# AechPro/rlgym-ppo

Hardware: AMD Instinct MI355X
Metric: ppo_update_samples_per_sec (higher is better)
Workload: dtype f32; 1 GPU; configs[1]: 4096 agents x 128 steps = 524,288-sample buffer, obs 107 f32, 90 discrete actions, 256x3 policy + critic; batch 524,288, minibatch 65,536

## Files before the change

rlgym_ppo_amd/csrc/api.hip:

```cpp
#include "build_id.h"
#include <math.h>
#include <stdarg.h>
#include <string.h>

#include "common.hpp"

namespace rlppo {

static thread_local char g_err[512] = "";

void set_error(const char *fmt, ...) {
    va_list ap;
    va_start(ap, fmt);
    vsnprintf(g_err, sizeof(g_err), fmt, ap);
    va_end(ap);
}

static int64_t padded_width(int64_t d) {
    const int64_t p16 = round_up(d, 16), p64 = round_up(d, 64);
    return (p64 - p16) * 10 >= p64 ? p16 : p64;
}
static int64_t padded_out(int64_t d) {
    if (d <= 32) return 32;
    if (d <= 64) return 64;
// ... 546 lines not shown
}

int64_t rlppo_act_done_words(int64_t n) { return n > 0 ? cdiv(n, 16) : 0; }

size_t rlppo_gae_workspace_bytes(int64_t n) { return gae_workspace_bytes(n) + 256; }

int rlppo_gae(void *stream, const float *rews, const float *dones, const float *truncated, const float *values, int64_t n,
              double gamma, double lmbda, float return_std, float *value_targets, float *advantages, float *returns,
              void *workspace, size_t ws_bytes) {
    if (n == 0) return 0;
    RLPPO_CHECK_ARG(n > 0 && rews && dones && truncated && values && value_targets && advantages && returns && workspace,
                    "gae: bad argument");
    return launch_gae((hipStream_t)stream, rews, dones, truncated, values, n, gamma, lmbda, return_std, value_targets,
                      advantages, returns, workspace, ws_bytes);
}

static int g_two_streams = 1;
static int g_fused_gather = 1;
static int g_update_bf16 = 0;
struct SlotBank {
    hipStream_t main[RLPPO_MAX_SLOTS] = {}, side[RLPPO_MAX_SLOTS] = {};
    hipEvent_t ev_fork[RLPPO_MAX_SLOTS] = {}, ev_join[RLPPO_MAX_SLOTS] = {}, ev_slot[RLPPO_MAX_SLOTS] = {}, ev_mid[RLPPO_MAX_SLOTS] = {};
    bool pending[RLPPO_MAX_SLOTS] = {};
};
static SlotBank g_banks[64];
static int slot_bank(SlotBank **bank) {
    int dev = 0;
    RLPPO_HIP(hipGetDevice(&dev));
    RLPPO_CHECK_ARG(dev >= 0 && dev < 64, "device id %d", dev);
    *bank = &g_banks[dev];
    return 0;
}
static int ensure_slot(SlotBank &b, int s) {
    if (!b.side[s]) {
        RLPPO_HIP(hipStreamCreateWithFlags(&b.side[s], hipStreamNonBlocking));
        RLPPO_HIP(hipStreamCreateWithFlags(&b.main[s], hipStreamNonBlocking));
        RLPPO_HIP(hipEventCreateWithFlags(&b.ev_fork[s], hipEventDisableTiming));
        RLPPO_HIP(hipEventCreateWithFlags(&b.ev_join[s], hipEventDisableTiming));
        RLPPO_HIP(hipEventCreateWithFlags(&b.ev_slot[s], hipEventDisableTiming));
        RLPPO_HIP(hipEventCreateWithFlags(&b.ev_mid[s], hipEventDisableTiming));
    }
    return 0;
}
static int order_after(hipStream_t to, hipStream_t from, hipEvent_t ev) {
    RLPPO_HIP(hipEventRecord(ev, from));
    RLPPO_HIP(hipStreamWaitEvent(to, ev, 0));
    return 0;
}

static size_t tn_layer_floats(const NetLayout &net, int l, int64_t mb, int prec) {
    size_t f = tn_partial_floats(net.L[l].out, net.L[l].in, mb);
    if (net.L[l].out == 1) {
        const size_t g = (size_t)cdiv(mb, 64) * (size_t)(net.L[l].pin + 4);
        if (g > f) f = g;
    }
    if (prec == 1 && l == net.n_layers - 1) {
        const size_t g = thin_dw_ws_floats(net.L[l].out, net.L[l].pin, mb);
        if (g > f) f = g;
    }
    return (f + 3) / 4 * 4;
}
static size_t tn_ws_floats(const NetLayout &net, int64_t mb, int prec) {
    size_t m = 0;
// ... 606 lines not shown
        rc = order_after(p.st, caller, bk.ev_slot[slot]);
        if (rc) return rc;
        bk.pending[slot] = true;
    }
    rc = gather(p);
    if (rc) return rc;
    p.side = p.st;
    if (g_two_streams) {
        p.side = bk.side[slot];
        rc = order_after(p.side, p.st, bk.ev_fork[slot]);
        if (rc) return rc;
    }
    ++g_cnt_pass;
    if (twin) ++g_cnt_paired_pass;
    if (p.rows.rowtab) ++g_cnt_gather_fused_pass;
    rc = twin ? paired_pass(p, bk, slot) : two_chain_pass(p);
    if (rc) return rc;
    if (!twin && p.side != p.st) {
        rc = order_after(p.st, p.side, bk.ev_join[slot]);
        if (rc) return rc;
    }
    if (p.defer && dws.n) {
        ++g_cnt_group_dw;
        rc = launch_gemm_tn_group(p.st, dws.p, dws.n, mb, p.w.pol.tn, p.w.tn_floats);
    }
    return rc;
}

int rlppo_ppo_join(void *stream) {
    SlotBank *bank = nullptr;
    int rc = slot_bank(&bank);
    if (rc) return rc;
    SlotBank &bk = *bank;
    for (int s = 1; s < RLPPO_MAX_SLOTS; ++s)
        if (bk.pending[s]) {
            rc = order_after((hipStream_t)stream, bk.main[s], bk.ev_slot[s]);
            if (rc) return rc;
            bk.pending[s] = false;
        }
    return 0;
}

int rlppo_clip_adam(void *stream, float *params, float *grads, float *exp_avg, float *exp_avg_sq, int64_t n,
                    double max_norm, double lr, double beta1, double beta2, double eps, int64_t step, double *gnorm2) {
    if (n == 0) return 0;
    RLPPO_CHECK_ARG(n > 0 && params && grads && exp_avg && exp_avg_sq && gnorm2 && step >= 1, "clip_adam: bad argument");
    const double bc1 = 1.0 - pow(beta1, (double)step);
// ... 146 lines not shown
    ++g_selection_epoch;
    return 0;
}
int rlppo_dbg_set(int32_t key, int32_t value) {
    ++g_selection_epoch;
    switch (key) {
        case 1: set_gae_algo(value); return 0;
        case 4: g_two_streams = value; return 0;
        case 21: set_gae_spin_limit(value); return 0;
        case 22: set_gae_oversubscribe(value); return 0;
        case 34: set_fused_spin_limit(value); return 0;
        case 35: set_fused_test_hold(value); return 0;
        case 36: set_split_persistent(value); return 0;
        case 23: set_b16_wide_tiles(value); return 0;
        case 24: set_exp_fast_transform(value); return 0;
        case 26: g_fused_gather = value; return 0;
        case 27: g_fused_act = value; return 0;
        case 29: g_paired = value; return 0;
        case 31: g_head_order = value; return 0;
        case 32: g_fold_vhead = value; return 0;
        case 33: set_pair_interleave(value); return 0;
        case 37: g_group_dw = value; return 0;
        case 38: set_tn_group_budget(value); return 0;
        case 40: set_nt_skinny(value); return 0;
        case 41: g_window_mode = value; return 0;
        default: break;
    }
    set_error("dbg_set: unknown key %d", key);
    return RLPPO_ERR_ARG;
}
int64_t rlppo_selection_epoch(void) { return g_selection_epoch; }
const int64_t *rlppo_selection_epoch_ptr(void) { return &g_selection_epoch; }
int64_t rlppo_dbg_counter(int32_t key) {
    switch (key) {
        case 0: return g_cnt_fused_act;
        case 1: return g_cnt_act_chain;
        case 2: return g_cnt_pass;
        case 3: return g_cnt_paired_pass;
        case 4: return g_cnt_gather_fused_pass;
        case 5: return g_cnt_group_dw;
        default: return -1;
    }
}
size_t rlppo_dbg_gemm_nt_bits_bytes(int64_t M, int32_t N) { return nt_bits_floats(M, N) * sizeof(float); }
int rlppo_dbg_gemm_nt_bits(void *stream, const float *A, int64_t lda, const float *B, int64_t ldb, const float *bias, float *C,
                           int64_t ldc, int64_t M, int32_t N, int32_t K, int32_t epilogue, void *bits) {
// ... 34 lines not shown
                            (float *)ws, ws_bytes / sizeof(float));
    return rc == -1 ? RLPPO_ERR_ARG : rc;
}
static int tn_products(const rlppo_tn_product *p, int32_t n, TnProduct *q) {
    RLPPO_CHECK_ARG(p && n > 0 && n <= 2 * RLPPO_MAX_LAYERS, "gemm_tn_group: %d products (1..%d)", n, 2 * RLPPO_MAX_LAYERS);
    for (int i = 0; i < n; ++i) {
        q[i].dY = p[i].dY; q[i].ldy = p[i].ldy; q[i].ny_valid = p[i].ny_valid; q[i].X = p[i].X; q[i].ldx = p[i].ldx;
        q[i].kx_valid = p[i].kx_valid; q[i].dW = p[i].dW; q[i].db = p[i].db; q[i].out = p[i].out; q[i].in = p[i].in;
        q[i].rowtab = p[i].rowtab; q[i].src_rows = p[i].src_rows;
    }
    return 0;
}
size_t rlppo_dbg_gemm_tn_group_workspace_bytes(const rlppo_tn_product *p, int32_t n, int64_t M) {
    if (!p || n <= 0 || n > 2 * RLPPO_MAX_LAYERS) return 0;
    int outs[2 * RLPPO_MAX_LAYERS], ins[2 * RLPPO_MAX_LAYERS];
    for (int i = 0; i < n; ++i) {
        outs[i] = p[i].out;
        ins[i] = p[i].in;
    }
    return tn_group_floats(outs, ins, n, M) * sizeof(float);
}
int rlppo_dbg_gemm_tn_group(void *stream, const rlppo_tn_product *p, int32_t n, int64_t M, void *ws, size_t ws_bytes) {
    TnProduct q[2 * RLPPO_MAX_LAYERS];
    const int rc = tn_products(p, n, q);
    if (rc) return rc;
    return launch_gemm_tn_group((hipStream_t)stream, q, n, M, (float *)ws, ws_bytes / sizeof(float));
}
size_t rlppo_dbg_gemm_tn_workspace_bytes(int32_t out, int32_t in, int64_t M) { return tn_partial_floats(out, in, M) * sizeof(float); }
int rlppo_dbg_gemm_tn(void *stream, const float *dY, int64_t ldy, int32_t ny_valid, const float *X, int64_t ldx,
                      int32_t kx_valid, float *dW, float *db, int32_t out, int32_t in, int64_t M, void *ws, size_t ws_bytes) {
    return launch_gemm_tn((hipStream_t)stream, dY, ldy, ny_valid, X, ldx, kx_valid, dW, db, out, in, M, (float *)ws,
                          ws_bytes / sizeof(float));
}
}
```

rlgym_ppo_amd/csrc/common.hpp:

```cpp
#pragma once
#include <hip/hip_runtime.h>
#include <stdint.h>
#include <stdio.h>

#include <atomic>

#include "../../include/rlppo.h"

namespace rlppo {

void set_error(const char *fmt, ...);

#define RLPPO_CHECK_ARG(cond, ...)                \
    do {                                          \
        if (!(cond)) {                            \
            rlppo::set_error(__VA_ARGS__);        \
            return RLPPO_ERR_ARG;                 \
        }                                         \
    } while (0)

#define RLPPO_HIP(expr)                                                                         \
    do {                                                                                        \
        hipError_t e_ = (expr);                                                                 \
        if (e_ != hipSuccess) {                                                                 \
// ... 84 lines not shown
void set_infer_bf16(int v);
void set_pair_interleave(int v);
void set_nt_skinny(int on);
int get_infer_bf16();
size_t tn_partial_floats(int out, int in, int64_t M);
int launch_gemm_tn(hipStream_t st, const float *dY, int64_t ldy, int ny_valid, const float *X, int64_t ldx, int kx_valid,
                   float *dW, float *db, int out, int in, int64_t M, float *ws, size_t ws_floats, const unsigned *rowtab = nullptr,
                   int64_t src_rows = 0, const TnPair *pair = nullptr);
bool tn_gather_ok(int64_t ldx, int64_t src_rows);
struct TnProduct {
    const float *dY = nullptr;
    int64_t ldy = 0;
    int ny_valid = 0;
    const float *X = nullptr;
    int64_t ldx = 0;
    int kx_valid = 0;
    float *dW = nullptr, *db = nullptr;
    int out = 0, in = 0;
    const unsigned *rowtab = nullptr;
    int64_t src_rows = 0;
};
constexpr int TN_GROUP_MAX = 2 * RLPPO_MAX_LAYERS;
size_t tn_group_floats(const int *outs, const int *ins, int n, int64_t M);
int launch_gemm_tn_group(hipStream_t st, const TnProduct *prods, int n, int64_t M, float *ws, size_t ws_floats);
void set_tn_group_budget(int workgroups);

bool nt_b16_ok(int N, int K, bool hidden);
bool nt_split_ok(int N, int K);
void set_split_persistent(int v);
int launch_pack_split(hipStream_t st, const float *S, int64_t ld, int R, int Cc, unsigned short *planes);
int launch_gemm_nt_split(hipStream_t st, const float *A, int64_t lda, const unsigned short *planes, const float *bias, float *C, int64_t ldc,
                         int64_t M, int N, int K, int mode, unsigned long long *bits);
int launch_gemm_nt_b16(hipStream_t st, const unsigned short *A, int64_t lda, const unsigned short *B, int64_t ldb, const float *bias,
                       float *C, int64_t ldc, unsigned short *Cb, int64_t ldcb, int64_t M, int N, int K, int epi, int mode,
                       unsigned long long *bits);
void set_b16_wide_tiles(int on);
bool tn_b16_ok(int pout, int pin);
int launch_gemm_tn_b16(hipStream_t st, const unsigned short *dY, int64_t ldy, const unsigned short *X, int64_t ldx, float *dW,
                       float *db, int pout, int pin, int out, int in, int64_t M, float *ws, size_t ws_floats);

void set_exp_fast_transform(int on);

bool gemv_head_ok(int out, int kp);
int launch_gemv_fwd(hipStream_t st, const float *x, int64_t ldx, const float *w, const float *b, float *y, int64_t ldy, int64_t n, int kp, int pout);
int launch_gemv_fwd_b16(hipStream_t st, const unsigned short *x, int64_t ldx, const float *w, const float *b, float *y, int64_t ldy,
                        int64_t n, int kp, int pout);
bool thin_head_ok(int out, int kp);
// ... 119 lines not shown
```

rlgym_ppo_amd/csrc/gemm.hip:

```cpp
#include "gemm_detail.hpp"

namespace rlppo {

template <int NB, int EPI, int BKT, bool BITS = false, bool GATHER = false>
__global__ __launch_bounds__(256, BKT == 16 ? 4 : 2) void gemm_nt_dma_kernel(const float *__restrict__ A, unsigned lda_b,
                                                                              const float *__restrict__ B, unsigned ldb_b,
                                                                              const float *__restrict__ bias,
                                                                              const float *__restrict__ mask_src,
                                                                              unsigned ldm_b, float *__restrict__ C,
                                                                              unsigned ldc_b, int64_t M, int K,
                                                                              unsigned long long *__restrict__ bits = nullptr,
                                                                              const unsigned *__restrict__ rowtab = nullptr,
                                                                              unsigned src_rows = 0, NtAlt alt = NtAlt{},
                                                                              NtDot dot = NtDot{}, NtDot dot_alt = NtDot{}) {
    constexpr int BN = NB * 16;
    constexpr int CPR = BKT / 4;
    constexpr int RPW = 64 / CPR;
    constexpr int RPP = 4 * RPW;
    constexpr int A_IT = SBM / RPP, B_IT = BN / RPP;
    constexpr int B_REM = BN % RPP;
    static_assert(B_REM % RPW == 0, "the ragged staging pass must be whole wave instructions");
    __shared__ __attribute__((aligned(16))) float lds[2 * SBM * BKT + 2 * BN * BKT];
    float *As = lds;
    float *Bs = lds + 2 * SBM * BKT;
// ... 461 lines not shown
        case 4: return launch_nt_1<4>(st, grid, epi, A, la, B, lb, bias, mask_src, lm, C, lc, M, K);
        default: return launch_nt_1<2>(st, grid, epi, A, la, B, lb, bias, mask_src, lm, C, lc, M, K);
    }
}

namespace {
constexpr int TM = 32;
constexpr unsigned OOR = 0x80000000u;
}

struct TnGeom {
    int ni, nj, wn;
    __host__ __device__ int bnt() const { return wn * ni * 16; }
    __host__ __device__ int bkx() const { return (4 / wn) * nj * 16; }
    __host__ __device__ int tile_floats() const { return ni * nj * 1024; }
};
static TnGeom tn_geometry(int out, int in) {
    if (in > 96 && in <= 112) return TnGeom{2, 7, 4};
    if (out > 64 && out <= 96) return TnGeom{3, 4, 2};
    return TnGeom{4, 4, 2};
}

constexpr int TN_LDS_FLOATS = 2 * 2 * 32 * 128;
template <int TMT, int NI, int NJ, int WN, bool GATHER>
__device__ __forceinline__ void tn_tile(float *lds, const float *__restrict__ dY, unsigned ldy_b, int ny_valid,
                                        const float *__restrict__ X, unsigned ldx_b, int kx_valid, bool with_db, int out, int64_t M,
                                        int rows_per_wg, float *__restrict__ partial, const unsigned *__restrict__ rowtab,
                                        unsigned src_rows, int bx, int by, int bz, int tiles_x, int tiles_y, int splits_z) {
    constexpr int WK = 4 / WN;
    constexpr int BNT = WN * NI * 16, BKX = WK * NJ * 16, TILE_F = NI * NJ * 1024;
    constexpr int PPW = TMT / 8;
    static_assert(2 * 2 * TMT * 128 <= TN_LDS_FLOATS && 8 * 128 <= TN_LDS_FLOATS, "stage buffers");
    float *Ys = lds;
    float *Xs = lds + 2 * TMT * 128;

    const int tid = threadIdx.x;
    const int lane = tid & 63, wave = tid >> 6;
    const int wave_u = __builtin_amdgcn_readfirstlane(wave);
    const int r16 = lane & 15, q = lane >> 4;
    const int wn = wave / WK, wk = wave % WK;
    const int n0 = bx * BNT, k0 = by * BKX;
    const int64_t mbeg = (int64_t)bz * rows_per_wg;
    const int rows = (int)((M - mbeg) < rows_per_wg ? (M - mbeg) : rows_per_wg);
    const int steps = (rows + TMT - 1) / TMT;
    const int rem = rows - (steps - 1) * TMT;
    const int ny_here = (ny_valid - n0) < BNT ? (ny_valid - n0) : BNT;
    const int kx_here = (kx_valid - k0) < BKX ? (kx_valid - k0) : BKX;

    const __amdgpu_buffer_rsrc_t y_rs = make_rsrc(reinterpret_cast<const char *>(dY) + mbeg * ldy_b + (int64_t)n0 * 4,
                                                  (unsigned)(rows - 1) * ldy_b + (unsigned)ny_here * 4);
    const __amdgpu_buffer_rsrc_t x_rs =
// ... 82 lines not shown
        for (int c = 0; c < TMT / 16; ++c) {
#pragma unroll
            for (int s = 0; s < 4; ++s) {
                const int m = c * 16 + s * 4;
                float fa[NI], fb[NJ];
#pragma unroll
                for (int i = 0; i < NI; ++i) fa[i] = Yc[m * 128 + fy[i]];
#pragma unroll
                for (int j = 0; j < NJ; ++j) fb[j] = Xc[m * 128 + fx[j]];
#pragma unroll
                for (int i = 0; i < NI; ++i)
#pragma unroll
                    for (int j = 0; j < NJ; ++j) {
                        if (c & 1) acc2[i][j] = MFMA16(fa[i], fb[j], acc2[i][j]);
                        else acc[i][j] = MFMA16(fa[i], fb[j], acc[i][j]);
                    }
            }
        }
        __builtin_amdgcn_sched_barrier(0);
        asm volatile("s_waitcnt vmcnt(0)" ::: "memory");
        if (more && (st + 2) == steps && rem < TMT) clear_tail(cur ^ 1);
        __syncthreads();
    }

    if (want_db) {
        float *red = lds;
        const int lcol = ((tid & 31) ^ ((zr & 3) << 2)) * 4;
        *reinterpret_cast<f32x4 *>(&red[zr * 128 + lcol]) = bs4;
        __syncthreads();
        if (tid < BNT && (n0 + tid) < out) {
            float sum = 0.f;
#pragma unroll
            for (int r = 0; r < 8; ++r) sum += red[r * 128 + tid];
            partial[(size_t)splits_z * tiles_y * tiles_x * TILE_F + ((size_t)bz * tiles_x + bx) * 128 + tid] = sum;
        }
    }
#pragma unroll
    for (int i = 0; i < NI; ++i)
#pragma unroll
        for (int j = 0; j < NJ; ++j) acc[i][j] += acc2[i][j];
    __builtin_amdgcn_sched_barrier(0);
    {
        const size_t tile_id = (size_t)bz * (tiles_x * tiles_y) + (size_t)by * tiles_x + bx;
        const __amdgpu_buffer_rsrc_t p_rs = make_rsrc(partial + tile_id * TILE_F, TILE_F * 4);
#pragma unroll
        for (int i = 0; i < NI; ++i)
#pragma unroll
            for (int j = 0; j < NJ; ++j) stb(p_rs, (unsigned)tid * 16, (unsigned)(i * NJ + j) * 4096, acc[i][j]);
    }
}

template <int TMT, int NI, int NJ, int WN, bool GATHER>
__global__ __launch_bounds__(256, 2) void gemm_tn_dma_kernel(const float *__restrict__ dY, unsigned ldy_b,
                                                                              int ny_valid, const float *__restrict__ X,
                                                                              unsigned ldx_b, int kx_valid,
                                                                              bool with_db, int out, int in, int64_t M,
                                                                              int rows_per_wg, float *__restrict__ partial,
                                                                              const unsigned *__restrict__ rowtab,
                                                                              unsigned src_rows, TnAlt alt) {
    __shared__ __attribute__((aligned(16))) float lds[TN_LDS_FLOATS];
    const int splits_z = alt.dY ? gridDim.z / 2 : gridDim.z;
    int zloc = blockIdx.z;
    bool second = alt.dY && !alt.interleave && zloc >= splits_z;
    if (second) zloc -= splits_z;
    int il_tile = -1, il_split = 0;
    if (alt.dY && alt.interleave) {
        const int T = gridDim.x * gridDim.y;
        const int id = (blockIdx.z * gridDim.y + blockIdx.y) * gridDim.x + blockIdx.x, g = id % (16 * T);
        int t2 = g >> 3;
        second = t2 >= T;
        if (second) t2 -= T;
        il_tile = t2;
        il_split = (id / (16 * T)) * 8 + (g & 7);
    }
    if (second) {
        dY = alt.dY;
        if (!GATHER) X = alt.X;
        partial = alt.partial;
    }
    int bx = blockIdx.x, by = blockIdx.y, bz = zloc;
    {
        const int T = gridDim.x * gridDim.y;
        if (il_tile >= 0) {
            bz = il_split;
            bx = il_tile % gridDim.x;
            by = il_tile / gridDim.x;
        } else if ((splits_z & 7) == 0 && T > 1) {
            const int id = (zloc * gridDim.y + blockIdx.y) * gridDim.x + blockIdx.x, g = id % (8 * T);
            const int tile = g >> 3;
            bz = (id / (8 * T)) * 8 + (g & 7);
            bx = tile % gridDim.x;
            by = tile / gridDim.x;
        }
    }
    tn_tile<TMT, NI, NJ, WN, GATHER>(lds, dY, ldy_b, ny_valid, X, ldx_b, kx_valid, with_db, out, M, rows_per_wg, partial, rowtab, src_rows,
                                     bx, by, bz, (int)gridDim.x, (int)gridDim.y, splits_z);
}


__device__ __forceinline__ void tn_reduce_tile(const float *__restrict__ partial, int splits, int tiles_x, int tiles,
                                               float *__restrict__ dW, float *__restrict__ db, int out, int in, TnGeom geo, int tile,
                                               int bxi, int nbx, float (*red)[64][4], float *dbh) {
    const int e64 = threadIdx.x & 63, sl = threadIdx.x >> 6;
    const int elem4 = bxi * 64 + e64;
    const int tile4 = geo.tile_floats() / 4;
    const f32x4 *base = reinterpret_cast<const f32x4 *>(partial) + (size_t)tile * tile4 + elem4;
    const size_t stride = (size_t)tiles * tile4;
    f32x4 acc = f32x4{0.f, 0.f, 0.f, 0.f};
    int sp = sl;
    for (; sp + 28 < splits; sp += 32) {
        f32x4 v[8];
#pragma unroll
        for (int u = 0; u < 8; ++u) v[u] = __builtin_nontemporal_load(base + (size_t)(sp + 4 * u) * stride);
#pragma unroll
        for (int u = 0; u < 8; ++u) acc += v[u];
    }
    for (; sp + 12 < splits; sp += 16) {
        f32x4 v[4];
#pragma unroll
        for (int u = 0; u < 4; ++u) v[u] = __builtin_nontemporal_load(base + (size_t)(sp + 4 * u) * stride);
#pragma unroll
        for (int u = 0; u < 4; ++u) acc += v[u];
    }
    for (; sp < splits; sp += 4) acc += __builtin_nontemporal_load(base + (size_t)sp * stride);
    if (sl > 0) *reinterpret_cast<f32x4 *>(&red[sl - 1][e64][0]) = acc;
    const int bnt = geo.bnt(), bkx = geo.bkx();
    const bool db_block = db && bxi == nbx - 1 && tile < tiles_x;
    float sdb = 0.f;
    if (db_block) {
        const int c = threadIdx.x & 127, half = threadIdx.x >> 7;
        const float *pdb = partial + (size_t)splits * tiles * geo.tile_floats() + (size_t)tile * 128 + c;
        const size_t dstride = (size_t)tiles_x * 128;
        const int s_lo = half ? (splits + 1) / 2 : 0, s_hi = half ? splits : (splits + 1) / 2;
        float a16[16];
#pragma unroll
        for (int u = 0; u < 16; ++u) a16[u] = 0.f;
        int s2 = s_lo;
        if (c < bnt) {
            for (; s2 + 15 < s_hi; s2 += 16) {
                float v[16];
#pragma unroll
                for (int u = 0; u < 16; ++u) v[u] = pdb[(size_t)(s2 + u) * dstride];
#pragma unroll
                for (int u = 0; u < 16; ++u) a16[u] += v[u];
            }
            for (int u = 0; s2 < s_hi; ++s2, ++u) a16[u] += pdb[(size_t)s2 * dstride];
        }
#pragma unroll
        for (int u = 0; u < 16; ++u) sdb += a16[u];
        if (half) dbh[c] = sdb;
    }
    __syncthreads();
    if (db_block && threadIdx.x < bnt && tile * bnt + (int)threadIdx.x < out)
        atomicAdd(db + tile * bnt + threadIdx.x, sdb + dbh[threadIdx.x]);
    if (sl > 0) return;
#pragma unroll
    for (int r = 0; r < 3; ++r) acc += *reinterpret_cast<const f32x4 *>(&red[r][e64][0]);
    const int ij = elem4 >> 8, t = elem4 & 255;
    const int i = ij / geo.nj, j = ij % geo.nj, wave = t >> 6, lane = t & 63;
    const int wkc = 4 / geo.wn, wn = wave / wkc, wk = wave % wkc;
    const int n0 = (tile % tiles_x) * bnt, k0 = (tile / tiles_x) * bkx;
    const int k = k0 + (wk * geo.nj + j) * 16 + (lane & 15);
    const int nb = n0 + (wn * geo.ni + i) * 16 + (lane >> 4) * 4;
    if (k < in) {
#pragma unroll
        for (int e = 0; e < 4; ++e)
            if (nb + e < out) atomicAdd(dW + (size_t)(nb + e) * in + k, acc[e]);
    }
}

__global__ __launch_bounds__(256) void tn_reduce_kernel(const float *__restrict__ partial, int splits, int tiles_x, int tiles,
                                                        float *__restrict__ dW, float *__restrict__ db, int out, int in,
                                                        TnGeom geo, TnRedAlt alt) {
    if (blockIdx.z) {
        partial = alt.partial;
        dW = alt.dW;
        db = alt.db;
    }
    __shared__ __attribute__((aligned(16))) float red[3][64][4];
    __shared__ float dbh[128];
    tn_reduce_tile(partial, splits, tiles_x, tiles, dW, db, out, in, geo, (int)blockIdx.y, (int)blockIdx.x, (int)gridDim.x, red, dbh);
}

static int64_t tn_rows_for(int64_t tiles, int64_t M) {
    int64_t rows = tiles >= 2 ? 512 : 256;
    if (M < 64 * rows) rows = round_up(cdiv(M, 64) > 32 ? cdiv(M, 64) : 32, 32);
    const int64_t few = round_up(cdiv(M * tiles, 512), 32);
    return few > rows ? few : rows;
}
int64_t tn_partial_rows(int out, int in, int64_t M) {
    return tn_rows_for(cdiv(out, 128) * cdiv(in, 128), M);
// ... 47 lines not shown
    if (g.nj == 7) {
        if (rowtab) TN(2, 7, 4, true); else TN(2, 7, 4, false);
    } else if (g.ni == 3) {
        RLPPO_CHECK_ARG(!rowtab, "gemm_tn (gathered rows): the 96-row tile has no gathered form");
        TN(3, 4, 2, false);
    } else {
        if (rowtab) TN(4, 4, 2, true); else TN(4, 4, 2, false);
    }
#undef TN
    RLPPO_LAUNCH_CHECK();
    TnRedAlt ralt{};
    if (pair) ralt = TnRedAlt{pair->ws, pair->dW, pair->db};
    return launch_tn_reduce(st, ws, splits, tiles_x, tiles_y, dW, db, out, in, g.ni, g.nj, g.wn, pair ? &ralt : nullptr);
}
int launch_tn_reduce(hipStream_t st, const float *partial, int splits, int tiles_x, int tiles_y, float *dW, float *db, int out, int in,
                     int ni, int nj, int wn, const TnRedAlt *alt) {
    hipLaunchKernelGGL(tn_reduce_kernel, dim3((unsigned)(ni * nj * 4), (unsigned)(tiles_x * tiles_y), alt ? 2u : 1u), dim3(256), 0, st,
                       partial, splits, tiles_x, tiles_x * tiles_y, dW, db, out, in, TnGeom{ni, nj, wn}, alt ? *alt : TnRedAlt{});
    RLPPO_LAUNCH_CHECK();
    return 0;
}
struct TnWork {
    const float *dY, *X;
    float *partial;
    const unsigned *rowtab;
    unsigned ldy_b, ldx_b, src_rows;
    int ny_valid, kx_valid, out, rows_per_wg, splits, tiles_x, tiles_y, with_db, geom, wg_begin;
};
struct TnGroupArgs {
    int n;
    int64_t M;
    TnWork w[TN_GROUP_MAX];
};
__global__ __launch_bounds__(256, 2) void gemm_tn_group_kernel(TnGroupArgs g) {
    __shared__ __attribute__((aligned(16))) float lds[TN_LDS_FLOATS];
    const int id = blockIdx.x;
    int p = 0;
    for (int i = 1; i < g.n; ++i)
        if (id >= g.w[i].wg_begin) p = i;
    const TnWork &w = g.w[p];
    const int loc = id - w.wg_begin, T = w.tiles_x * w.tiles_y, S8 = w.splits & ~7;
    int tile, bz;
    if (loc < S8 * T) {
        const int gq = loc % (8 * T);
        tile = gq >> 3;
        bz = (loc / (8 * T)) * 8 + (gq & 7);
    } else {
        const int r = loc - S8 * T, R = w.splits - S8;
        if (R <= 0 || r >= R * T) return;
        tile = r / R;
        bz = S8 + r % R;
    }
    const int bx = tile % w.tiles_x, by = tile / w.tiles_x;
#define TN_ITEM(NI_, NJ_, WN_, G_)                                                                                                     \
    tn_tile<TM, NI_, NJ_, WN_, G_>(lds, w.dY, w.ldy_b, w.ny_valid, w.X, w.ldx_b, w.kx_valid, w.with_db != 0, w.out, g.M, w.rows_per_wg, \
                                   w.partial, w.rowtab, w.src_rows, bx, by, bz, w.tiles_x, w.tiles_y, w.splits)
    switch (w.geom) {
        case 0: TN_ITEM(4, 4, 2, false); break;
        case 1: TN_ITEM(4, 4, 2, true); break;
        case 2: TN_ITEM(3, 4, 2, false); break;
        case 3: TN_ITEM(2, 7, 4, false); break;
        default: TN_ITEM(2, 7, 4, true); break;
    }
#undef TN_ITEM
}

struct TnRedWork {
    const float *partial;
    float *dW, *db;
    int splits, tiles_x, tiles, out, in, tile_begin;
    TnGeom geo;
};
struct TnRedGroupArgs {
    int n;
    TnRedWork w[TN_GROUP_MAX];
};
__global__ __launch_bounds__(256) void tn_reduce_group_kernel(TnRedGroupArgs g) {
    __shared__ __attribute__((aligned(16))) float red[3][64][4];
    __shared__ float dbh[128];
    const int t = blockIdx.y;
    int p = 0;
    for (int i = 1; i < g.n; ++i)
        if (t >= g.w[i].tile_begin) p = i;
    const TnRedWork &w = g.w[p];
    const int nbx = w.geo.ni * w.geo.nj * 4;
    if ((int)blockIdx.x >= nbx) return;
    tn_reduce_tile(w.partial, w.splits, w.tiles_x, w.tiles, w.dW, w.db, w.out, w.in, w.geo, t - w.tile_begin, (int)blockIdx.x, nbx, red, dbh);
}

static int g_tn_group_budget = 0;
constexpr int TN_MAX_CHAIN = 8192;
void set_tn_group_budget(int v) { g_tn_group_budget = v; }
struct TnPlanItem {
    TnGeom g;
    int tiles_x, tiles_y, splits, rows_per_wg, wg_begin;
    size_t partial_off, floats;
};
static int tn_group_plan(const int *outs, const int *ins, int n, int64_t M, int budget, TnPlanItem *it, int *total_wgs, size_t *total_floats) {
    for (int p = 0; p < n; ++p) {
        it[p].g = tn_geometry(outs[p], ins[p]);
        it[p].tiles_x = (int)cdiv(outs[p], it[p].g.bnt());
        it[p].tiles_y = (int)cdiv(ins[p], it[p].g.bkx());
    }
    const int64_t max_splits = cdiv(M, 32);
    auto fill = [&](double t) {
        int64_t wgs = 0;
        for (int p = 0; p < n; ++p) {
            const int blocks = it[p].g.ni * it[p].g.nj;
            int64_t rows = (int64_t)(t / blocks);
            rows = round_up(rows < 32 ? 32 : rows, 32);
            if (g_tn_group_budget <= 0 && rows > TN_MAX_CHAIN) rows = TN_MAX_CHAIN;
            int64_t sp = cdiv(M, rows);
            if (sp > max_splits) sp = max_splits;
            rows = round_up(cdiv(M, sp), 32);
            it[p].rows_per_wg = (int)rows;
            it[p].splits = (int)cdiv(M, rows);
            wgs += round_up((int64_t)it[p].splits * it[p].tiles_x * it[p].tiles_y, 8);
        }
        return wgs;
    };
    for (int rounds = g_tn_group_budget > 0 ? 1 : 2;; ++rounds) {
        const int64_t cap = (int64_t)budget * rounds;
        double lo = 32.0, hi = (double)round_up(M, 32) * 32.0;
        if (fill(lo) <= cap) break;
        for (int i = 0; i < 60; ++i) {
            const double mid = 0.5 * (lo + hi);
            if (fill(mid) > cap) lo = mid; else hi = mid;
        }
        if (fill(hi) <= cap || g_tn_group_budget > 0 || rounds >= 256) break;
    }
    int wg = 0;
    size_t off = 0;
    for (int p = 0; p < n; ++p) {
        it[p].wg_begin = wg;
        wg += (int)round_up((int64_t)it[p].splits * it[p].tiles_x * it[p].tiles_y, 8);
        it[p].partial_off = off;
        it[p].floats = (size_t)it[p].splits * it[p].tiles_x * it[p].tiles_y * (size_t)it[p].g.tile_floats() + (size_t)it[p].splits * it[p].tiles_x * 128;
        off += (it[p].floats + 3) / 4 * 4;
    }
    *total_wgs = wg;
    *total_floats = off;
    return 0;
}
static int tn_group_budget() {
    if (g_tn_group_budget > 0) return g_tn_group_budget;
    int cus = 0;
    if (device_cu_count(&cus) || cus <= 0) cus = 256;
    return 2 * cus;
}
size_t tn_group_floats(const int *outs, const int *ins, int n, int64_t M) {
    if (n <= 0 || M <= 0) return 0;
    size_t total = 0;
    for (int b = 0; b < n; b += TN_GROUP_MAX) {
        TnPlanItem it[TN_GROUP_MAX];
        int wgs = 0;
        size_t f = 0;
        const int m = n - b < TN_GROUP_MAX ? n - b : TN_GROUP_MAX;
        tn_group_plan(outs + b, ins + b, m, M, tn_group_budget(), it, &wgs, &f);
        total = f > total ? f : total;
    }
    return total;
}
int launch_gemm_tn_group(hipStream_t st, const TnProduct *prods, int n, int64_t M, float *ws, size_t ws_floats) {
    if (M <= 0 || n <= 0) return 0;
    for (int b = 0; b < n; b += TN_GROUP_MAX) {
        const int m = n - b < TN_GROUP_MAX ? n - b : TN_GROUP_MAX;
        const TnProduct *pr = prods + b;
        int outs[TN_GROUP_MAX], ins[TN_GROUP_MAX];
        for (int p = 0; p < m; ++p) {
            outs[p] = pr[p].out;
            ins[p] = pr[p].in;
        }
        TnPlanItem it[TN_GROUP_MAX];
        int wgs = 0;
        size_t floats = 0;
        tn_group_plan(outs, ins, m, M, tn_group_budget(), it, &wgs, &floats);
        if (!ws || ws_floats < floats) {
            set_error("gemm_tn_group: workspace %zu < %zu floats", ws ? ws_floats : (size_t)0, floats);
            return RLPPO_ERR_WORKSPACE;
        }
        TnGroupArgs ga{};
        TnRedGroupArgs ra{};
        ga.n = ra.n = m;
        ga.M = M;
        const int64_t lim = (int64_t)1 << 30;
        int tile_begin = 0;
        for (int p = 0; p < m; ++p) {
            const TnProduct &q = pr[p];
            RLPPO_CHECK_ARG(q.dY && q.X && q.dW && q.ny_valid % 4 == 0 && q.kx_valid % 4 == 0 && q.ldy % 4 == 0 && q.ldx % 4 == 0 &&
                                q.ny_valid <= q.ldy && q.kx_valid <= q.ldx && q.out <= q.ny_valid && q.in <= q.kx_valid,
                            "gemm_tn_group: bad shapes (product %d) ny=%d kx=%d ldy=%ld ldx=%ld out=%d in=%d", p, q.ny_valid, q.kx_valid,
                            (long)q.ldy, (long)q.ldx, q.out, q.in);
            RLPPO_CHECK_ARG(((int64_t)it[p].rows_per_wg + TM) * q.ldy * 4 < lim && (q.rowtab || ((int64_t)it[p].rows_per_wg + TM) * q.ldx * 4 < lim),
                            "gemm_tn_group: a leading dimension is too wide for 32-bit tile offsets");
            RLPPO_CHECK_ARG(!q.rowtab || tn_gather_ok(q.ldx, q.src_rows), "gemm_tn_group (gathered rows): unsupported row stride %ld", (long)q.ldx);
            RLPPO_CHECK_ARG(!(q.rowtab && it[p].g.ni == 3), "gemm_tn_group (gathered rows): the 96-row tile has no gathered form");
            TnWork &w = ga.w[p];
            w.dY = q.dY;
            w.X = q.X;
            w.partial = ws + it[p].partial_off;
            w.rowtab = q.rowtab;
            w.ldy_b = (unsigned)(q.ldy * 4);
            w.ldx_b = (unsigned)(q.ldx * 4);
            w.src_rows = (unsigned)q.src_rows;
            w.ny_valid = q.ny_valid;
            w.kx_valid = q.kx_valid;
            w.out = q.out;
            w.rows_per_wg = it[p].rows_per_wg;
            w.splits = it[p].splits;
            w.tiles_x = it[p].tiles_x;
            w.tiles_y = it[p].tiles_y;
            w.with_db = q.db != nullptr;
            w.geom = it[p].g.nj == 7 ? (q.rowtab ? 4 : 3) : it[p].g.ni == 3 ? 2 : (q.rowtab ? 1 : 0);
            w.wg_begin = it[p].wg_begin;
            TnRedWork &r = ra.w[p];
            r.partial = w.partial;
            r.dW = q.dW;
            r.db = q.db;
            r.splits = it[p].splits;
            r.tiles_x = it[p].tiles_x;
            r.tiles = it[p].tiles_x * it[p].tiles_y;
            r.out = q.out;
            r.in = q.in;
            r.tile_begin = tile_begin;
            r.geo = it[p].g;
            tile_begin += r.tiles;
        }
        hipLaunchKernelGGL(gemm_tn_group_kernel, dim3((unsigned)wgs), dim3(256), 0, st, ga);
        RLPPO_LAUNCH_CHECK();
        hipLaunchKernelGGL(tn_reduce_group_kernel, dim3(64u, (unsigned)tile_begin), dim3(256), 0, st, ra);
        RLPPO_LAUNCH_CHECK();
    }
    return 0;
}
}
```

Before: 61.13 million samples/s.

## Make grouped weight-gradient GEMM persistent with atomic work stealing and slow-first ordering

Adds a persistent form of the grouped TN (weight-gradient) GEMM kernel. A capped grid of workgroups draws further work items from device atomic counters, and the slowest tile geometries are ordered first. This form is used by default when there are at least 262144 rows. An optional form 1 fuses the split-K reduction, where the last workgroup to finish a tile reduces it via ticket counters, but the default form 3 still launches the separate reduce kernel. The aim is to remove tail imbalance and the cost of launching many short-lived workgroups, at the price of atomic traffic, cache-bypassing partial stores and a per-slot sync buffer.

```diff
diff --git a/rlgym_ppo_amd/csrc/api.hip b/rlgym_ppo_amd/csrc/api.hip
--- a/rlgym_ppo_amd/csrc/api.hip
+++ b/rlgym_ppo_amd/csrc/api.hip
@@ -592,6 +592,7 @@
     hipStream_t main[RLPPO_MAX_SLOTS] = {}, side[RLPPO_MAX_SLOTS] = {};
     hipEvent_t ev_fork[RLPPO_MAX_SLOTS] = {}, ev_join[RLPPO_MAX_SLOTS] = {}, ev_slot[RLPPO_MAX_SLOTS] = {}, ev_mid[RLPPO_MAX_SLOTS] = {};
     bool pending[RLPPO_MAX_SLOTS] = {};
+    unsigned *tn_sync[RLPPO_MAX_SLOTS + 1] = {};
 };
 static SlotBank g_banks[64];
 static int slot_bank(SlotBank **bank) {
@@ -609,6 +610,16 @@
         RLPPO_HIP(hipEventCreateWithFlags(&b.ev_join[s], hipEventDisableTiming));
         RLPPO_HIP(hipEventCreateWithFlags(&b.ev_slot[s], hipEventDisableTiming));
         RLPPO_HIP(hipEventCreateWithFlags(&b.ev_mid[s], hipEventDisableTiming));
+    }
+    return 0;
+}
+static int ensure_tn_sync(SlotBank &b, int s) {
+    if (!b.tn_sync[s]) {
+        unsigned *blk = nullptr;
+        RLPPO_HIP(hipMalloc(&blk, TN_SYNC_WORDS * sizeof(unsigned)));
+        RLPPO_HIP(hipMemset(blk, 0, TN_SYNC_WORDS * sizeof(unsigned)));
+        RLPPO_HIP(hipDeviceSynchronize());
+        b.tn_sync[s] = blk;
     }
     return 0;
 }
@@ -1261,7 +1272,9 @@
     }
     if (p.defer && dws.n) {
         ++g_cnt_group_dw;
-        rc = launch_gemm_tn_group(p.st, dws.p, dws.n, mb, p.w.pol.tn, p.w.tn_floats);
+        rc = ensure_tn_sync(bk, slot);
+        if (rc) return rc;
+        rc = launch_gemm_tn_group(p.st, dws.p, dws.n, mb, p.w.pol.tn, p.w.tn_floats, bk.tn_sync[slot]);
     }
     return rc;
 }
@@ -1454,6 +1467,7 @@
         case 33: set_pair_interleave(value); return 0;
         case 37: g_group_dw = value; return 0;
         case 38: set_tn_group_budget(value); return 0;
+        case 42: set_tn_group_form(value); return 0;
         case 40: set_nt_skinny(value); return 0;
         case 41: g_window_mode = value; return 0;
         default: break;
@@ -1534,9 +1548,14 @@
 }
 int rlppo_dbg_gemm_tn_group(void *stream, const rlppo_tn_product *p, int32_t n, int64_t M, void *ws, size_t ws_bytes) {
     TnProduct q[2 * RLPPO_MAX_LAYERS];
-    const int rc = tn_products(p, n, q);
-    if (rc) return rc;
-    return launch_gemm_tn_group((hipStream_t)stream, q, n, M, (float *)ws, ws_bytes / sizeof(float));
+    int rc = tn_products(p, n, q);
+    if (rc) return rc;
+    SlotBank *bank = nullptr;
+    rc = slot_bank(&bank);
+    if (rc) return rc;
+    rc = ensure_tn_sync(*bank, RLPPO_MAX_SLOTS);
+    if (rc) return rc;
+    return launch_gemm_tn_group((hipStream_t)stream, q, n, M, (float *)ws, ws_bytes / sizeof(float), bank->tn_sync[RLPPO_MAX_SLOTS]);
 }
 size_t rlppo_dbg_gemm_tn_workspace_bytes(int32_t out, int32_t in, int64_t M) { return tn_partial_floats(out, in, M) * sizeof(float); }
 int rlppo_dbg_gemm_tn(void *stream, const float *dY, int64_t ldy, int32_t ny_valid, const float *X, int64_t ldx,
diff --git a/rlgym_ppo_amd/csrc/common.hpp b/rlgym_ppo_amd/csrc/common.hpp
--- a/rlgym_ppo_amd/csrc/common.hpp
+++ b/rlgym_ppo_amd/csrc/common.hpp
@@ -130,7 +130,9 @@
 };
 constexpr int TN_GROUP_MAX = 2 * RLPPO_MAX_LAYERS;
 size_t tn_group_floats(const int *outs, const int *ins, int n, int64_t M);
-int launch_gemm_tn_group(hipStream_t st, const TnProduct *prods, int n, int64_t M, float *ws, size_t ws_floats);
+constexpr int TN_SYNC_TICKETS = 4096, TN_SYNC_WORDS = 16 + TN_SYNC_TICKETS;
+int launch_gemm_tn_group(hipStream_t st, const TnProduct *prods, int n, int64_t M, float *ws, size_t ws_floats, unsigned *sync);
+void set_tn_group_form(int form);
 void set_tn_group_budget(int workgroups);
 
 bool nt_b16_ok(int N, int K, bool hidden);
diff --git a/rlgym_ppo_amd/csrc/gemm.hip b/rlgym_ppo_amd/csrc/gemm.hip
--- a/rlgym_ppo_amd/csrc/gemm.hip
+++ b/rlgym_ppo_amd/csrc/gemm.hip
@@ -507,11 +507,11 @@
 }
 
 constexpr int TN_LDS_FLOATS = 2 * 2 * 32 * 128;
-template <int TMT, int NI, int NJ, int WN, bool GATHER>
+template <int TMT, int NI, int NJ, int WN, bool GATHER, int ST_AUX, class Pre>
 __device__ __forceinline__ void tn_tile(float *lds, const float *__restrict__ dY, unsigned ldy_b, int ny_valid,
                                         const float *__restrict__ X, unsigned ldx_b, int kx_valid, bool with_db, int out, int64_t M,
                                         int rows_per_wg, float *__restrict__ partial, const unsigned *__restrict__ rowtab,
-                                        unsigned src_rows, int bx, int by, int bz, int tiles_x, int tiles_y, int splits_z) {
+                                        unsigned src_rows, int bx, int by, int bz, int tiles_x, int tiles_y, int splits_z, Pre pre) {
     constexpr int WK = 4 / WN;
     constexpr int BNT = WN * NI * 16, BKX = WK * NJ * 16, TILE_F = NI * NJ * 1024;
     constexpr int PPW = TMT / 8;
@@ -640,6 +640,7 @@
         if (more && (st + 2) == steps && rem < TMT) clear_tail(cur ^ 1);
         __syncthreads();
     }
+    pre();
 
     if (want_db) {
         float *red = lds;
@@ -650,7 +651,9 @@
             float sum = 0.f;
 #pragma unroll
             for (int r = 0; r < 8; ++r) sum += red[r * 128 + tid];
-            partial[(size_t)splits_z * tiles_y * tiles_x * TILE_F + ((size_t)bz * tiles_x + bx) * 128 + tid] = sum;
+            float *dst = partial + (size_t)splits_z * tiles_y * tiles_x * TILE_F + ((size_t)bz * tiles_x + bx) * 128 + tid;
+            if (ST_AUX) __hip_atomic_store(dst, sum, __ATOMIC_RELAXED, __HIP_MEMORY_SCOPE_AGENT);
+            else *dst = sum;
         }
     }
 #pragma unroll
@@ -664,7 +667,8 @@
 #pragma unroll
         for (int i = 0; i < NI; ++i)
 #pragma unroll
-            for (int j = 0; j < NJ; ++j) stb(p_rs, (unsigned)tid * 16, (unsigned)(i * NJ + j) * 4096, acc[i][j]);
+            for (int j = 0; j < NJ; ++j)
+                __builtin_amdgcn_raw_buffer_store_b128(__builtin_bit_cast(u32x4, acc[i][j]), p_rs, (unsigned)tid * 16, (unsigned)(i * NJ + j) * 4096, ST_AUX);
     }
 }
 
@@ -711,11 +715,31 @@
             by = tile / gridDim.x;
         }
     }
-    tn_tile<TMT, NI, NJ, WN, GATHER>(lds, dY, ldy_b, ny_valid, X, ldx_b, kx_valid, with_db, out, M, rows_per_wg, partial, rowtab, src_rows,
-                                     bx, by, bz, (int)gridDim.x, (int)gridDim.y, splits_z);
-}
-
-
+    tn_tile<TMT, NI, NJ, WN, GATHER, 0>(lds, dY, ldy_b, ny_valid, X, ldx_b, kx_valid, with_db, out, M, rows_per_wg, partial, rowtab, src_rows,
+                                     bx, by, bz, (int)gridDim.x, (int)gridDim.y, splits_z, [] {});
+}
+
+
+__device__ __forceinline__ float tn_db_half(const float *pdb, size_t dstride, int s_lo, int s_hi, bool written) {
+    float a16[16];
+#pragma unroll
+    for (int u = 0; u < 16; ++u) a16[u] = 0.f;
+    int s2 = s_lo;
+    if (written) {
+        for (; s2 + 15 < s_hi; s2 += 16) {
+            float v[16];
+#pragma unroll
+            for (int u = 0; u < 16; ++u) v[u] = pdb[(size_t)(s2 + u) * dstride];
+#pragma unroll
+            for (int u = 0; u < 16; ++u) a16[u] += v[u];
+        }
+        for (int u = 0; s2 < s_hi; ++s2, ++u) a16[u] += pdb[(size_t)s2 * dstride];
+    }
+    float sdb = 0.f;
+#pragma unroll
+    for (int u = 0; u < 16; ++u) sdb += a16[u];
+    return sdb;
+}
 __device__ __forceinline__ void tn_reduce_tile(const float *__restrict__ partial, int splits, int tiles_x, int tiles,
                                                float *__restrict__ dW, float *__restrict__ db, int out, int in, TnGeom geo, int tile,
                                                int bxi, int nbx, float (*red)[64][4], float *dbh) {
@@ -750,22 +774,7 @@
         const float *pdb = partial + (size_t)splits * tiles * geo.tile_floats() + (size_t)tile * 128 + c;
         const size_t dstride = (size_t)tiles_x * 128;
         const int s_lo = half ? (splits + 1) / 2 : 0, s_hi = half ? splits : (splits + 1) / 2;
-        float a16[16];
-#pragma unroll
-        for (int u = 0; u < 16; ++u) a16[u] = 0.f;
-        int s2 = s_lo;
-        if (c < bnt) {
-            for (; s2 + 15 < s_hi; s2 += 16) {
-                float v[16];
-#pragma unroll
-                for (int u = 0; u < 16; ++u) v[u] = pdb[(size_t)(s2 + u) * dstride];
-#pragma unroll
-                for (int u = 0; u < 16; ++u) a16[u] += v[u];
-            }
-            for (int u = 0; s2 < s_hi; ++s2, ++u) a16[u] += pdb[(size_t)s2 * dstride];
-        }
-#pragma unroll
-        for (int u = 0; u < 16; ++u) sdb += a16[u];
+        sdb = tn_db_half(pdb, dstride, s_lo, s_hi, c < bnt);
         if (half) dbh[c] = sdb;
     }
     __syncthreads();
@@ -785,6 +794,79 @@
         for (int e = 0; e < 4; ++e)
             if (nb + e < out) atomicAdd(dW + (size_t)(nb + e) * in + k, acc[e]);
     }
+}
+
+__device__ __forceinline__ void tn_reduce_whole_tile(const float *__restrict__ partial, int splits, int tiles_x, int tiles,
+                                                     float *__restrict__ dW, float *__restrict__ db, int out, int in, TnGeom geo, int tile,
+                                                     float *dbh) {
+    const int tid = threadIdx.x, wave = tid >> 6, lane = tid & 63;
+    const int tile4 = geo.tile_floats() / 4, nblk = geo.ni * geo.nj;
+    const size_t stride = (size_t)tiles * tile4;
+    const int bnt = geo.bnt(), bkx = geo.bkx();
+    const int wkc = 4 / geo.wn, wn = wave / wkc, wk = wave % wkc;
+    const int n0 = (tile % tiles_x) * bnt, k0 = (tile / tiles_x) * bkx;
+    const f32x4 z = f32x4{0.f, 0.f, 0.f, 0.f};
+    for (int ij = 0; ij < nblk; ij += 2) {
+        const bool two = ij + 1 < nblk;
+        const f32x4 *base[2];
+        base[0] = reinterpret_cast<const f32x4 *>(partial) + (size_t)tile * tile4 + ij * 256 + tid;
+        base[1] = base[0] + (two ? 256 : 0);
+        f32x4 a[2][4];
+#pragma unroll
+        for (int e = 0; e < 2; ++e)
+#pragma unroll
+            for (int u = 0; u < 4; ++u) a[e][u] = z;
+        int sp = 0;
+        for (; sp + 7 < splits; sp += 8) {
+            f32x4 v[2][8];
+#pragma unroll
+            for (int e = 0; e < 2; ++e)
+#pragma unroll
+                for (int u = 0; u < 8; ++u) v[e][u] = __builtin_nontemporal_load(base[e] + (size_t)(sp + u) * stride);
+#pragma unroll
+            for (int e = 0; e < 2; ++e)
+#pragma unroll
+                for (int u = 0; u < 8; ++u) a[e][u & 3] += v[e][u];
+        }
+        for (; sp < splits; sp += 4) {
+            f32x4 v[2][4];
+#pragma unroll
+            for (int e = 0; e < 2; ++e)
+#pragma unroll
+                for (int u = 0; u < 4; ++u) v[e][u] = sp + u < splits ? __builtin_nontemporal_load(base[e] + (size_t)(sp + u) * stride) : z;
+#pragma unroll
+            for (int e = 0; e < 2; ++e)
+#pragma unroll
+                for (int u = 0; u < 4; ++u)
+                    if (sp + u < splits) a[e][u] += v[e][u];
+        }
+#pragma unroll
+        for (int e = 0; e < 2; ++e) {
+            if (e && !two) break;
+            f32x4 acc = a[e][0];
+#pragma unroll
+            for (int u = 1; u < 4; ++u) acc += a[e][u];
+            const int i = (ij + e) / geo.nj, j = (ij + e) % geo.nj;
+            const int k = k0 + (wk * geo.nj + j) * 16 + (lane & 15);
+            const int nb = n0 + (wn * geo.ni + i) * 16 + (lane >> 4) * 4;
+            if (k < in) {
+#pragma unroll
+                for (int c = 0; c < 4; ++c)
+                    if (nb + c < out) atomicAdd(dW + (size_t)(nb + c) * in + k, acc[c]);
+            }
+        }
+    }
+    const bool with_db = db && tile < tiles_x;
+    float sdb = 0.f;
+    if (with_db) {
+        const int c = tid & 127, half = tid >> 7;
+        const float *pdb = partial + (size_t)splits * tiles * geo.tile_floats() + (size_t)tile * 128 + c;
+        const int s_lo = half ? (splits + 1) / 2 : 0, s_hi = half ? splits : (splits + 1) / 2;
+        sdb = tn_db_half(pdb, (size_t)tiles_x * 128, s_lo, s_hi, c < bnt);
+        if (half) dbh[c] = sdb;
+    }
+    __syncthreads();
+    if (with_db && tid < bnt && tile * bnt + tid < out) atomicAdd(db + tile * bnt + tid, sdb + dbh[tid]);
 }
 
 __global__ __launch_bounds__(256) void tn_reduce_kernel(const float *__restrict__ partial, int splits, int tiles_x, int tiles,
@@ -878,48 +960,145 @@
 }
 struct TnWork {
     const float *dY, *X;
-    float *partial;
+    float *partial, *dW, *db;
     const unsigned *rowtab;
     unsigned ldy_b, ldx_b, src_rows;
-    int ny_valid, kx_valid, out, rows_per_wg, splits, tiles_x, tiles_y, with_db, geom, wg_begin;
+    int ny_valid, kx_valid, out, in, rows_per_wg, splits, tiles_x, tiles_y, with_db, geom, wg_begin, ticket_begin;
+    TnGeom geo;
 };
 struct TnGroupArgs {
-    int n;
+    int n, total;
+    int form;
     int64_t M;
+    unsigned *sync;
     TnWork w[TN_GROUP_MAX];
 };
-__global__ __launch_bounds__(256, 2) void gemm_tn_group_kernel(TnGroupArgs g) {
+#ifndef TN_SC1
+#define TN_SC1 1
+#endif
+#ifdef TN_TRACE
+constexpr int TN_TRACE_ITEMS = 8192;
+__device__ unsigned g_tn_trace[TN_TRACE_ITEMS][8];
+__device__ __forceinline__ void tn_trace_item(int id, unsigned long long t_start, unsigned long long t_end, unsigned sum_ticks, int geom) {
+    if (threadIdx.x != 0 || id >= TN_TRACE_ITEMS) return;
+    unsigned *t = g_tn_trace[id];
+    t[0] = (unsigned)t_start;
+    t[1] = (unsigned)(t_start >> 32);
+    t[2] = (unsigned)t_end;
+    t[3] = (unsigned)(t_end >> 32);
+    t[4] = sum_ticks;
+    t[5] = __builtin_amdgcn_s_getreg((31 << 11) | 4);
+    t[6] = __builtin_amdgcn_s_getreg((31 << 11) | 20);
+    t[7] = (unsigned)(geom + 1);
+}
+#endif
+__device__ __forceinline__ bool tn_group_item(const TnWork &w, int id, int &tile, int &bz) {
+    const int loc = id - w.wg_begin, T = w.tiles_x * w.tiles_y, S8 = w.splits & ~7;
+    if (loc < S8 * T) {
+        const int gq = loc % (8 * T);
+        tile = gq >> 3;
+        bz = (loc / (8 * T)) * 8 + (gq & 7);
+        return true;
+    }
+    const int r = loc - S8 * T, R = w.splits - S8;
+    if (R <= 0 || r >= R * T) return false;
+    tile = r / R;
+    bz = S8 + r % R;
+    return true;
+}
+#define TN_ITEM(NI_, NJ_, WN_, G_, AUX_, PRE_)                                                                                              \
+    tn_tile<TM, NI_, NJ_, WN_, G_, AUX_>(lds, w.dY, w.ldy_b, w.ny_valid, w.X, w.ldx_b, w.kx_valid, w.with_db != 0, w.out, g.M, w.rows_per_wg, \
+                                         w.partial, w.rowtab, w.src_rows, bx, by, bz, w.tiles_x, w.tiles_y, w.splits, PRE_)
+#define TN_ITEM_SWITCH(AUX_, PRE_)                          \
+    switch (w.geom) {                                       \
+        case 0: TN_ITEM(4, 4, 2, false, AUX_, PRE_); break; \
+        case 1: TN_ITEM(4, 4, 2, true, AUX_, PRE_); break;  \
+        case 2: TN_ITEM(3, 4, 2, false, AUX_, PRE_); break; \
+        case 3: TN_ITEM(2, 7, 4, false, AUX_, PRE_); break; \
+        default: TN_ITEM(2, 7, 4, true, AUX_, PRE_); break; \
+    }
+__global__ __launch_bounds__(256, 2) void gemm_tn_group_item_kernel(TnGroupArgs g) {
     __shared__ __attribute__((aligned(16))) float lds[TN_LDS_FLOATS];
+#ifdef TN_TRACE
+    const unsigned long long t_start = wall_clock64();
+#endif
     const int id = blockIdx.x;
     int p = 0;
     for (int i = 1; i < g.n; ++i)
         if (id >= g.w[i].wg_begin) p = i;
     const TnWork &w = g.w[p];
-    const int loc = id - w.wg_begin, T = w.tiles_x * w.tiles_y, S8 = w.splits & ~7;
     int tile, bz;
-    if (loc < S8 * T) {
-        const int gq = loc % (8 * T);
-        tile = gq >> 3;
-        bz = (loc / (8 * T)) * 8 + (gq & 7);
-    } else {
-        const int r = loc - S8 * T, R = w.splits - S8;
-        if (R <= 0 || r >= R * T) return;
-        tile = r / R;
-        bz = S8 + r % R;
-    }
+    if (!tn_group_item(w, id, tile, bz)) return;
     const int bx = tile % w.tiles_x, by = tile / w.tiles_x;
-#define TN_ITEM(NI_, NJ_, WN_, G_)                                                                                                     \
-    tn_tile<TM, NI_, NJ_, WN_, G_>(lds, w.dY, w.ldy_b, w.ny_valid, w.X, w.ldx_b, w.kx_valid, w.with_db != 0, w.out, g.M, w.rows_per_wg, \
-                                   w.partial, w.rowtab, w.src_rows, bx, by, bz, w.tiles_x, w.tiles_y, w.splits)
-    switch (w.geom) {
-        case 0: TN_ITEM(4, 4, 2, false); break;
-        case 1: TN_ITEM(4, 4, 2, true); break;
-        case 2: TN_ITEM(3, 4, 2, false); break;
-        case 3: TN_ITEM(2, 7, 4, false); break;
-        default: TN_ITEM(2, 7, 4, true); break;
-    }
+    TN_ITEM_SWITCH(0, [] {})
+#ifdef TN_TRACE
+    asm volatile("s_waitcnt vmcnt(0)" ::: "memory");
+    tn_trace_item(id, t_start, wall_clock64(), 0u, w.geom);
+#endif
+}
+__global__ __launch_bounds__(256, 2) void gemm_tn_group_kernel(TnGroupArgs g) {
+    __shared__ __attribute__((aligned(16))) float lds[TN_LDS_FLOATS];
+    __shared__ int s_next, s_last;
+    const int xr = blockIdx.x & 7;
+    unsigned drawn = 0;
+    auto draw = [&] {
+        if (threadIdx.x == 0) drawn = atomicAdd(g.sync + xr, 1u);
+    };
+    for (int id = blockIdx.x; id < g.total;) {
+#ifdef TN_TRACE
+        const unsigned long long t_start = wall_clock64();
+#endif
+        int p = 0;
+        for (int i = 1; i < g.n; ++i)
+            if (id >= g.w[i].wg_begin) p = i;
+        const TnWork &w = g.w[p];
+        int tile = -1, bz = 0;
+        const bool item = tn_group_item(w, id, tile, bz);
+        if (item) {
+            const int bx = tile % w.tiles_x, by = tile / w.tiles_x;
+            TN_ITEM_SWITCH(TN_SC1 ? 16 : 0, draw)
+        } else {
+            draw();
+        }
+        __builtin_amdgcn_sched_barrier(0);
+        asm volatile("s_waitcnt vmcnt(0)" ::: "memory");
+        __syncthreads();
+#ifdef TN_TRACE
+        const unsigned long long t_end = wall_clock64();
+#endif
+        if (threadIdx.x == 0) {
+            bool last = false;
+            if (g.form == 1 && item) {
+#if !TN_SC1
+                __builtin_amdgcn_fence(__ATOMIC_RELEASE, "agent");
+                asm volatile("s_waitcnt vmcnt(0)" ::: "memory");
+#endif
+                last = atomicAdd(g.sync + 16 + w.ticket_begin + tile, 1u) == (unsigned)w.splits - 1u;
+                if (last) {
+                    __builtin_amdgcn_fence(__ATOMIC_ACQUIRE, "agent");
+                    asm volatile("s_waitcnt vmcnt(0)" ::: "memory");
+                }
+            }
+            s_last = last;
+            s_next = (int)gridDim.x + 8 * (int)drawn + xr;
+        }
+        __syncthreads();
+        if (s_last) {
+            tn_reduce_whole_tile(w.partial, w.splits, w.tiles_x, w.tiles_x * w.tiles_y, w.dW, w.db, w.out, w.in, w.geo, tile, lds);
+            if (threadIdx.x == 0) __hip_atomic_store(g.sync + 16 + w.ticket_begin + tile, 0u, __ATOMIC_RELAXED, __HIP_MEMORY_SCOPE_AGENT);
+        }
+#ifdef TN_TRACE
+        if (item) tn_trace_item(id, t_start, t_end, s_last ? (unsigned)(wall_clock64() - t_end) : 0u, w.geom);
+#endif
+        id = s_next;
+        __syncthreads();
+    }
+    if (threadIdx.x == 0 && atomicAdd(g.sync + 8, 1u) == gridDim.x - 1) {
+        for (int i = 0; i <= 8; ++i) __hip_atomic_store(g.sync + i, 0u, __ATOMIC_RELAXED, __HIP_MEMORY_SCOPE_AGENT);
+    }
+}
+#undef TN_ITEM_SWITCH
 #undef TN_ITEM
-}
 
 struct TnRedWork {
     const float *partial;
@@ -945,14 +1124,17 @@
 }
 
 static int g_tn_group_budget = 0;
+static int g_tn_group_form = 2;
+void set_tn_group_form(int v) { g_tn_group_form = v; }
 constexpr int TN_MAX_CHAIN = 8192;
 void set_tn_group_budget(int v) { g_tn_group_budget = v; }
 struct TnPlanItem {
     TnGeom g;
-    int tiles_x, tiles_y, splits, rows_per_wg, wg_begin;
+    int tiles_x, tiles_y, splits, rows_per_wg, wg_begin, pos;
     size_t partial_off, floats;
 };
-static int tn_group_plan(const int *outs, const int *ins, int n, int64_t M, int budget, TnPlanItem *it, int *total_wgs, size_t *total_floats) {
+static int tn_group_plan(const int *outs, const int *ins, int n, int64_t M, int budget, TnPlanItem *it, int *total_wgs, size_t *total_floats,
+                         bool slow_first = false) {
     for (int p = 0; p < n; ++p) {
         it[p].g = tn_geometry(outs[p], ins[p]);
         it[p].tiles_x = (int)cdiv(outs[p], it[p].g.bnt());
@@ -985,11 +1167,17 @@
         }
         if (fill(hi) <= cap || g_tn_group_budget > 0 || rounds >= 256) break;
     }
-    int wg = 0;
+    int wg = 0, pos = 0;
+    for (int rank = 0; rank < 3; ++rank)
+        for (int p = 0; p < n; ++p) {
+            const int r = !slow_first ? 0 : it[p].g.nj == 7 ? 0 : it[p].g.ni == 3 ? 1 : 2;
+            if (r != rank) continue;
+            it[p].pos = pos++;
+            it[p].wg_begin = wg;
+            wg += (int)round_up((int64_t)it[p].splits * it[p].tiles_x * it[p].tiles_y, 8);
+        }
     size_t off = 0;
     for (int p = 0; p < n; ++p) {
-        it[p].wg_begin = wg;
-        wg += (int)round_up((int64_t)it[p].splits * it[p].tiles_x * it[p].tiles_y, 8);
         it[p].partial_off = off;
         it[p].floats = (size_t)it[p].splits * it[p].tiles_x * it[p].tiles_y * (size_t)it[p].g.tile_floats() + (size_t)it[p].splits * it[p].tiles_x * 128;
         off += (it[p].floats + 3) / 4 * 4;
@@ -1017,8 +1205,10 @@
     }
     return total;
 }
-int launch_gemm_tn_group(hipStream_t st, const TnProduct *prods, int n, int64_t M, float *ws, size_t ws_floats) {
+constexpr int64_t TN_PERSIST_MIN_ROWS = 262144;
+int launch_gemm_tn_group(hipStream_t st, const TnProduct *prods, int n, int64_t M, float *ws, size_t ws_floats, unsigned *sync) {
     if (M <= 0 || n <= 0) return 0;
+    const int want_form = !sync ? 0 : g_tn_group_form == 2 ? (M >= TN_PERSIST_MIN_ROWS ? 3 : 0) : g_tn_group_form;
     for (int b = 0; b < n; b += TN_GROUP_MAX) {
         const int m = n - b < TN_GROUP_MAX ? n - b : TN_GROUP_MAX;
         const TnProduct *pr = prods + b;
@@ -1030,7 +1220,10 @@
         TnPlanItem it[TN_GROUP_MAX];
         int wgs = 0;
         size_t floats = 0;
-        tn_group_plan(outs, ins, m, M, tn_group_budget(), it, &wgs, &floats);
+        int tiles = 0;
+        for (int p = 0; p < m; ++p) tiles += (int)(cdiv(outs[p], tn_geometry(outs[p], ins[p]).bnt()) * cdiv(ins[p], tn_geometry(outs[p], ins[p]).bkx()));
+        const int form = tiles <= TN_SYNC_TICKETS ? want_form : 0;
+        tn_group_plan(outs, ins, m, M, tn_group_budget(), it, &wgs, &floats, form != 0);
         if (!ws || ws_floats < floats) {
             set_error("gemm_tn_group: workspace %zu < %zu floats", ws ? ws_floats : (size_t)0, floats);
             return RLPPO_ERR_WORKSPACE;
@@ -1038,7 +1231,10 @@
         TnGroupArgs ga{};
         TnRedGroupArgs ra{};
         ga.n = ra.n = m;
+        ga.total = wgs;
         ga.M = M;
+        ga.form = form;
+        ga.sync = sync;
         const int64_t lim = (int64_t)1 << 30;
         int tile_begin = 0;
         for (int p = 0; p < m; ++p) {
@@ -1051,7 +1247,7 @@
                             "gemm_tn_group: a leading dimension is too wide for 32-bit tile offsets");
             RLPPO_CHECK_ARG(!q.rowtab || tn_gather_ok(q.ldx, q.src_rows), "gemm_tn_group (gathered rows): unsupported row stride %ld", (long)q.ldx);
             RLPPO_CHECK_ARG(!(q.rowtab && it[p].g.ni == 3), "gemm_tn_group (gathered rows): the 96-row tile has no gathered form");
-            TnWork &w = ga.w[p];
+            TnWork &w = ga.w[it[p].pos];
             w.dY = q.dY;
             w.X = q.X;
             w.partial = ws + it[p].partial_off;
@@ -1069,6 +1265,11 @@
             w.with_db = q.db != nullptr;
             w.geom = it[p].g.nj == 7 ? (q.rowtab ? 4 : 3) : it[p].g.ni == 3 ? 2 : (q.rowtab ? 1 : 0);
             w.wg_begin = it[p].wg_begin;
+            w.dW = q.dW;
+            w.db = q.db;
+            w.in = q.in;
+            w.geo = it[p].g;
+            w.ticket_begin = tile_begin;
             TnRedWork &r = ra.w[p];
             r.partial = w.partial;
             r.dW = q.dW;
@@ -1082,10 +1283,36 @@
             r.geo = it[p].g;
             tile_begin += r.tiles;
         }
-        hipLaunchKernelGGL(gemm_tn_group_kernel, dim3((unsigned)wgs), dim3(256), 0, st, ga);
+        int grid = wgs;
+        if (form != 0) {
+            grid = (int)round_up(tn_group_budget(), 8);
+            grid = grid < wgs ? grid : wgs;
+        }
+        if (form != 0) hipLaunchKernelGGL(gemm_tn_group_kernel, dim3((unsigned)grid), dim3(256), 0, st, ga);
+        else hipLaunchKernelGGL(gemm_tn_group_item_kernel, dim3((unsigned)grid), dim3(256), 0, st, ga);
         RLPPO_LAUNCH_CHECK();
-        hipLaunchKernelGGL(tn_reduce_group_kernel, dim3(64u, (unsigned)tile_begin), dim3(256), 0, st, ra);
-        RLPPO_LAUNCH_CHECK();
+        if (form != 1) {
+            hipLaunchKernelGGL(tn_reduce_group_kernel, dim3(64u, (unsigned)tile_begin), dim3(256), 0, st, ra);
+            RLPPO_LAUNCH_CHECK();
+        }
+#ifdef TN_TRACE
+        if (const char *path = getenv("RLPPO_TN_TRACE")) {
+            static unsigned host[TN_TRACE_ITEMS][8];
+            RLPPO_HIP(hipStreamSynchronize(st));
+            RLPPO_HIP(hipMemcpyFromSymbol(host, HIP_SYMBOL(g_tn_trace), sizeof(host)));
+            if (FILE *f = fopen(path, "ab")) {
+                const unsigned ids = wgs < TN_TRACE_ITEMS ? (unsigned)wgs : (unsigned)TN_TRACE_ITEMS;
+                const unsigned head[8] = {0x544e5452u, (unsigned)M, (unsigned)m, ids, (unsigned)form, (unsigned)grid, 0u, 0u};
+                fwrite(head, 4, 8, f);
+                for (int p = 0; p < m; ++p) {
+                    const unsigned pw[4] = {(unsigned)ga.w[p].geom, (unsigned)ga.w[p].splits, (unsigned)(ga.w[p].tiles_x * ga.w[p].tiles_y), (unsigned)ga.w[p].rows_per_wg};
+                    fwrite(pw, 4, 4, f);
+                }
+                fwrite(host, 32, ids, f);
+                fclose(f);
+            }
+        }
+#endif
     }
     return 0;
 }
```

Result: no change. 61.22 million samples/s, median of 2 (+0.1%).
